# BornToDeath/h264-h265-to-jpeg

Hardware: AMD Instinct MI355X
Metric: 1080p H.265 I-frames/sec → JPEG at 1/2/4/8 MI355X; achieved HBM GB/s vs peak (higher is better)
Workload: dtype u8

## Files before the change

h264-h265-to-jpeg_amd/csrc/host/cabac.h:

```cpp
#pragma once
#include <cstdint>

namespace h2j {

#ifdef H2J_CABAC_COUNT
extern thread_local unsigned long long g_bins_ctx, g_bins_byp;
#define H2J_COUNT(v, n) (v += (n))
#else
#define H2J_COUNT(v, n) ((void)0)
#endif

#pragma GCC visibility push(hidden)
extern const uint8_t kCabacLps[64][4];
extern const uint8_t kCabacTransLps[64];
extern const uint8_t kCabacRenorm[32];
extern const uint16_t kCabacNextMps[128];
extern const uint16_t kCabacNextLps[128];
extern const uint8_t kCabacLpsByState[128][8];
typedef uint64_t CabacState;
extern const uint64_t kCabacWord[128];

extern const uint64_t kCabacNextMpsW[128];
extern const uint64_t kCabacNextLpsW[128];
#pragma GCC visibility pop


inline uint8_t cabac_init_state(int m, int n, int qp) {
    if (qp < 0) qp = 0;
    if (qp > 51) qp = 51;
    int pre = ((m * qp) >> 4) + n;
    if (pre < 1) pre = 1;
    if (pre > 126) pre = 126;
    int mps = pre <= 63 ? 0 : 1;
    int st = mps ? pre - 64 : 63 - pre;
    return static_cast<uint8_t>((st << 1) | mps);
}
inline CabacState cabac_init_word(int m, int n, int qp) { return kCabacWord[cabac_init_state(m, n, qp)]; }

template <bool kInlineRefill>
class CabacT {
public:
    void init(const uint8_t* p, const uint8_t* end) {
        cur_ = p;
        end_ = end;
        range_ = 510;
        value_ = 0;
        for (int i = 0; i < 4; i++) value_ = (value_ << 8) | (cur_ < end_ ? *cur_++ : 0u);
        bits_ = 32 - 9;
    }
    __attribute__((always_inline)) inline int decision(CabacState& ctx) {
        H2J_COUNT(g_bins_ctx, 1);
        const uint64_t w = ctx;
        const unsigned st = static_cast<unsigned>(w >> 32);
        const uint32_t lps = static_cast<uint32_t>(w >> ((range_ >> 3) & 24)) & 0xffu;
        const uint32_t rmps = range_ - lps;
        const uint64_t scaled = static_cast<uint64_t>(rmps) << bits_;
        const uint32_t msh = (rmps >> 8) ^ 1u;
        uint32_t r = rmps << msh, sh = msh;
        const uint32_t lsh = static_cast<uint32_t>(__builtin_clz(lps)) - 23u;
        const uint32_t lr = lps << lsh;
        uint64_t nx = kCabacNextMpsW[st];
        const uint64_t nl = kCabacNextLpsW[st];
        uint64_t v = value_;
        const uint64_t vl = value_ - scaled;
        uint32_t is_lps = 0;
#if defined(__x86_64__)
        __asm__("cmpq %[sc], %[v]\n\t"
                "cmovaeq %[vl], %[v]\n\t"
                "cmovael %[lr], %[r]\n\t"
                "cmovael %[ls], %[sh]\n\t"
                "cmovaeq %[nl], %[nx]\n\t"
                "setae %b[il]"
                : [v] "+r"(v), [r] "+r"(r), [sh] "+r"(sh), [nx] "+r"(nx), [il] "+q"(is_lps)
                : [sc] "r"(scaled), [vl] "r"(vl), [lr] "r"(lr), [ls] "r"(lsh), [nl] "r"(nl)
                : "cc");
#else
        is_lps = v >= scaled ? 1u : 0u;
        v = is_lps ? vl : v;
        r = is_lps ? lr : r;
        sh = is_lps ? lsh : sh;
        nx = is_lps ? nl : nx;
#endif
        value_ = v;
        range_ = r;
        bits_ -= static_cast<int>(sh);
        ctx = nx;
        if (bits_ < 0) refill();
        return static_cast<int>((st & 1) ^ is_lps);
    }
    __attribute__((always_inline)) int bypass_b() {
        H2J_COUNT(g_bins_byp, 1);
        if (--bits_ < 0) refill();
// ... 106 lines not shown
```

h264-h265-to-jpeg_amd/csrc/host/hevc_parser.cpp:

```cpp
#include <algorithm>
#include <array>
#include <atomic>
#include <cstdlib>
#include <cstring>
#include <memory>
#include <thread>
#include <vector>

#include "bitstream.h"
#include "cabac.h"
#include "job.h"

namespace h2j {
#ifdef H2J_CORO
extern thread_local void (*g_h2j_yield)();
#endif
namespace {

enum {
    C_SAO_MERGE = 0, C_SAO_TYPE = 1, C_SPLIT_CU = 2, C_TQ_BYPASS = 5, C_PART_MODE = 6,
    C_PREV_INTRA = 7, C_CHROMA_MODE = 8, C_SPLIT_TF = 9, C_CBF_LUMA = 12, C_CBF_CHROMA = 14,
    C_TSKIP = 18, C_LAST_X = 20, C_LAST_Y = 38, C_CSBF = 56, C_SIG = 60, C_GT1 = 104,
    C_GT2 = 128, C_QP_DELTA = 134, C_CQO_FLAG = 136, C_CQO_IDX = 137, NUM_CTX = 138
};

const uint8_t kInitI[NUM_CTX] = {
    153, 200, 139, 141, 157, 154, 184, 184, 63, 153, 138, 138, 111, 141, 94, 138, 182, 154,
    139, 139,
    110, 110, 124, 125, 140, 153, 125, 127, 140, 109, 111, 143, 127, 111, 79, 108, 123, 63,
    110, 110, 124, 125, 140, 153, 125, 127, 140, 109, 111, 143, 127, 111, 79, 108, 123, 63,
    91, 171, 134, 141,
    111, 111, 125, 110, 110, 94, 124, 108, 124, 107, 125, 141, 179, 153, 125, 107, 125, 141,
    179, 153, 125, 107, 125, 141, 179, 153, 125, 140, 139, 182, 182, 152, 136, 152, 136, 153,
    136, 139, 111, 136, 139, 111, 141, 111,
    140, 92, 137, 138, 140, 152, 138, 139, 153, 74, 149, 92, 139, 107, 122, 152, 140, 179, 166,
    182, 140, 227, 122, 197,
    138, 153, 136, 167, 152, 152,
    154, 154,
    154, 154};

struct Sps {
    bool valid = false;
    int chroma_format_idc = 0, width = 0, height = 0;
    int conf_l = 0, conf_r = 0, conf_t = 0, conf_b = 0;
    int bit_depth = 8, bit_depth_c = 8, log2_max_poc_lsb = 4;
    int num_reorder_pics = 0;
    int log2_min_cb = 3, log2_ctb = 4, log2_min_tb = 2, log2_max_tb = 5, max_th_depth_intra = 0;
    int scaling_list_enabled = 0;
    uint8_t sl[4][6][64];
    uint8_t sl_dc[4][6];
    int sao = 0, pcm = 0, pcm_bd = 8, pcm_bd_c = 8, log2_min_pcm = 0, log2_max_pcm = 0, pcm_lf_disabled = 0;
    int num_st_rps = 0;
    int st_num_delta[65];
    int long_term_present = 0, num_lt_sps = 0, temporal_mvp = 0, strong_intra_smoothing = 0;
    int profile_idc = 0;
    int ts_rotation = 0, ts_context = 0, implicit_rdpcm = 0, explicit_rdpcm = 0, ext_precision = 0;
    int smoothing_disabled = 0, high_prec_offsets = 0, persistent_rice = 0, bypass_alignment = 0;
};

struct Pps {
    bool valid = false;
    int sps_id = 0, dependent_slices = 0, output_flag_present = 0, num_extra_bits = 0, sign_hiding = 0;
    int init_qp = 26, transform_skip = 0, cu_qp_delta = 0, diff_cu_qp_delta_depth = 0;
    int cb_qp_offset = 0, cr_qp_offset = 0, slice_chroma_qp_present = 0, transquant_bypass = 0;
    int tiles = 0, wpp = 0, ntc = 1, ntr = 1, uniform = 1, lf_across_tiles = 1;
    int col_w[64], row_h[64];
    int lf_across_slices = 0, deblock_override = 0, deblock_disabled = 0, beta_offset = 0, tc_offset = 0;
    int sl_present = 0;
    uint8_t sl[4][6][64];
    uint8_t sl_dc[4][6];
    int slice_header_ext = 0;
    int log2_max_ts = 2, cross_component = 0, cqo_list_enabled = 0, sao_scale_luma = 0, sao_scale_chroma = 0;
    int cqo_depth = 0, cqo_len_minus1 = 0, cb_qo[6] = {0, 0, 0, 0, 0, 0}, cr_qo[6] = {0, 0, 0, 0, 0, 0};
};

struct SliceHdr {
    int first_in_pic = 0, dependent = 0, address = 0, slice_addr_rs = 0, pps_id = 0, type = 0;
    int sao_luma = 0, sao_chroma = 0, qp_delta = 0, cb_qp_offset = 0, cr_qp_offset = 0;
    int deblock_disabled = 0, beta_offset = 0, tc_offset = 0, lf_across_slices = 0, slice_qp = 26;
    int cu_chroma_qp_offset_enabled = 0;
    std::vector<uint32_t> entry;
};

const uint8_t kSlIntra[64] = {
    16, 16, 16, 16, 16, 16, 16, 16, 16, 16, 17, 16, 17, 16, 17, 18, 17, 18, 18, 17, 18, 21,
    19, 20, 21, 20, 19, 21, 24, 22, 22, 24, 24, 22, 22, 24, 25, 25, 27, 30, 27, 25, 25, 29,
    31, 35, 35, 31, 29, 36, 41, 44, 41, 36, 47, 54, 54, 47, 65, 70, 65, 88, 88, 115};
const uint8_t kSlInter[64] = {
    16, 16, 16, 16, 16, 16, 16, 16, 16, 16, 17, 17, 17, 17, 17, 18, 18, 18, 18, 18, 18, 20,
    20, 20, 20, 20, 20, 20, 24, 24, 24, 24, 24, 24, 24, 24, 25, 25, 25, 25, 25, 25, 25, 28,
    28, 28, 28, 28, 28, 33, 33, 33, 33, 33, 41, 41, 41, 41, 54, 54, 54, 71, 71, 91};

void sl_default(uint8_t sl[4][6][64], uint8_t dc[4][6]) {
    for (int m = 0; m < 6; m++) {
        std::memset(sl[0][m], 16, 16);
        for (int s = 1; s < 4; s++) {
            std::memcpy(sl[s][m], m < 3 ? kSlIntra : kSlInter, 64);
            dc[s][m] = 16;
        }
// ... 445 lines not shown
        ctbs_ = proto.ctbs_;
    }
    int run(const uint8_t* data, size_t size, int threads);

private:
    HevcParser(const HevcParser&) = default;
    FrameJob* job_;
    std::vector<h2j_ctb>* ctbs_;
    Sps sps_[16];
    Pps pps_[64];
    const Sps* s_ = nullptr;
    const Pps* p_ = nullptr;
    std::vector<SliceHdr> sh_;
    std::vector<uint8_t> rbsp_;
    std::vector<uint8_t> slice_data_;
    int W = 0, H = 0, log2ctb = 0, ctbs = 0, ctbW = 0, ctbH = 0, nctb = 0, mw = 0, mh = 0;
    int qpbd = 0;
    std::vector<int8_t> qp_store_;
    std::vector<uint8_t> ipm_store_, ctd_store_;
    std::vector<int> addr_store_, slice_store_;
    int8_t* qp_ = nullptr;
    uint8_t *ipm_ = nullptr, *ctd_ = nullptr;
    int *ctb_addr_rs_ = nullptr, *ctb_slice_ = nullptr;
    void bind_maps() {
        qp_ = qp_store_.data();
        ipm_ = ipm_store_.data();
        ctd_ = ctd_store_.data();
        ctb_addr_rs_ = addr_store_.data();
        ctb_slice_ = slice_store_.data();
    }
    std::vector<int> rs2ts_, ts2rs_, tile_id_, col_bd_;
    const SliceHdr* cur_ = nullptr;
    int cur_idx_ = 0;
    Cabac cc_;
    const uint8_t* end_ = nullptr;
    CabacState ctx_[NUM_CTX], ctx_wpp_[NUM_CTX], ctx_ds_[NUM_CTX];
    int stat_[4] = {0, 0, 0, 0}, stat_wpp_[4] = {0, 0, 0, 0}, stat_ds_[4] = {0, 0, 0, 0};
    bool rext_ = false;
    bool have_ds_ = false;
    int qp_y_ = 0, qg_pred_ = 0, qpd_val_ = 0, last_cu_qp_ = 0;
    bool is_qpd_coded_ = false, first_qg_ = true;
    bool cqo_coded_ = false;
    int cu_qo_cb_ = 0, cu_qo_cr_ = 0;
    int cu_bypass_ = 0;
    int cu_tu_begin_ = 0;
    int err_ = 0;

    int parse_slice_header(BitReader& b, int nal_type, SliceHdr& sh, const SliceHdr* prev);
    bool setup_picture();
    bool setup_tiles();
    int decode_slice_data(int shi, const uint8_t* p, const uint8_t* end);
    struct WppRows;
    int decode_wpp_row(int shi, int row, const uint8_t* p, const uint8_t* end, WppRows& w);
    int run_wpp(const std::vector<uint8_t>& seg, const std::vector<uint32_t>& sub, int threads);
    int decode_tile(int shi, int ts0, int ts1, bool last, const uint8_t* p, const uint8_t* end);
    int run_tiles(const std::vector<uint8_t>& seg, const std::vector<uint32_t>& sub, int threads);
    void merge_parts(const std::vector<FrameJob>& part);
    void ctb_start_contexts(int rs, int ts, bool first);
    void init_contexts(int qp) {
        for (int i = 0; i < NUM_CTX; i++) {
            int iv = kInitI[i];
            ctx_[i] = cabac_init_word((iv >> 4) * 5 - 45, ((iv & 15) << 3) - 16, qp);
        }
        std::memset(stat_, 0, sizeof(stat_));
    }
    bool same_region(int xc, int yc, int xn, int yn) const {
        if (xn < 0 || yn < 0 || xn >= W || yn >= H) return false;
        if (((xn ^ xc) | (yn ^ yc)) >> log2ctb == 0) return true;
        int cn = (yn >> log2ctb) * ctbW + (xn >> log2ctb);
        int cc = (yc >> log2ctb) * ctbW + (xc >> log2ctb);
        if (tile_id_[rs2ts_[cn]] != tile_id_[rs2ts_[cc]] || ctb_slice_[cn] < 0) return false;
        return ctb_addr_rs_[cn] == ctb_addr_rs_[cc];
    }
    void qg_start(int xq, int yq);
    void parse_sao(int rx, int ry);
    void coding_quadtree(int x0, int y0, int log2cb, int depth);
    void coding_unit(int x0, int y0, int log2cb);
    void transform_tree(int x0, int y0, int xb, int yb, int log2n, int depth, int blk, int max_depth,
                        int intra_split, int pcb, int pcr, int cm, int cux, int cuy, int log2cb);
    void transform_unit(int x0, int y0, int xb, int yb, int log2n, int blk, int cbf_l, int cbf_cb,
                        int cbf_cr, int cm, int cux, int cuy, int log2cb);
    template <bool RExt>
    void residual(int log2n, int c, int mode, h2j_tu& tu);
    void emit_tu(int x, int y, int log2n, int c, int mode, uint8_t flags, bool cbf, int pred_mode_for_scan);
    void split_ctb_records(size_t first);
    std::vector<h2j_tu> chroma_tmp_;
    uint8_t edge_flags(int x0, int y0) const;
    void pcm_sample(int x0, int y0, int log2cb);
    int qp_wrap(int x) const {
        const int m = 52 + qpbd;
        if (static_cast<unsigned>(x) < static_cast<unsigned>(2 * m)) return x >= m ? x - m : x;
        return x % m;
    }
    static void fill_rows(uint8_t* p, int stride, int rows, int w, uint8_t v) {
        const uint64_t v8 = 0x0101010101010101ull * v;
        for (int y = 0; y < rows; y++, p += stride) {
            if (w == 2) std::memcpy(p, &v8, 2);
            else if (w == 4) std::memcpy(p, &v8, 4);
            else if (w == 8) std::memcpy(p, &v8, 8);
            else if (w == 16) { std::memcpy(p, &v8, 8); std::memcpy(p + 8, &v8, 8); }
            else std::memset(p, v, static_cast<size_t>(w));
        }
    }
    void set_map(uint8_t* m, int x0, int y0, int n, uint8_t v) {
        int ye = std::min((y0 + n) >> 2, mh), xe = std::min((x0 + n) >> 2, mw);
        fill_rows(&m[(y0 >> 2) * mw + (x0 >> 2)], mw, ye - (y0 >> 2), xe - (x0 >> 2), v);
    }
    void set_qp(int x0, int y0, int n, int qp) {
        int ye = std::min((y0 + n) >> 2, mh), xe = std::min((x0 + n) >> 2, mw);
        fill_rows(reinterpret_cast<uint8_t*>(&qp_[(y0 >> 2) * mw + (x0 >> 2)]), mw, ye - (y0 >> 2), xe - (x0 >> 2),
                  static_cast<uint8_t>(qp & 0xFF));
    }
    __attribute__((always_inline)) int dec(int ctx) { return cc_.decision(ctx_[ctx]); }
};

int HevcParser::parse_slice_header(BitReader& b, int nal_type, SliceHdr& sh, const SliceHdr* prev) {
    sh = SliceHdr();
    sh.first_in_pic = static_cast<int>(b.u(1));
    if (nal_type >= 16 && nal_type <= 23) b.u(1);
    const uint32_t pps_id = b.ue();
    if (pps_id > 63 || !pps_[pps_id].valid) return -1;
    sh.pps_id = static_cast<int>(pps_id);
    const Pps& p = pps_[sh.pps_id];
    if (p.sps_id > 15 || !sps_[p.sps_id].valid) return -1;
    const Sps& s = sps_[p.sps_id];
    if (!sh.first_in_pic) {
        if (p.dependent_slices) sh.dependent = static_cast<int>(b.u(1));
        int cs = 1 << s.log2_ctb;
        int n = ((s.width + cs - 1) / cs) * ((s.height + cs - 1) / cs);
        sh.address = static_cast<int>(b.u(ceil_log2(n)));
        if (sh.address >= n) return -1;
    }
    if (sh.dependent) {
        if (!prev) return -1;
        int addr = sh.address, first = sh.first_in_pic;
        sh = *prev;
        sh.address = addr;
        sh.dependent = 1;
        sh.first_in_pic = first;
    } else {
        sh.slice_addr_rs = sh.address;
        for (int i = 0; i < p.num_extra_bits; i++) b.u(1);
        sh.type = static_cast<int>(b.ue());
        if (p.output_flag_present) b.u(1);
        if (nal_type != 19 && nal_type != 20) {
            b.u(s.log2_max_poc_lsb);
            int sps_flag = static_cast<int>(b.u(1));
            if (!sps_flag) {
                Sps tmp = s;
                if (!parse_st_rps(b, tmp, s.num_st_rps)) return -1;
            } else if (s.num_st_rps > 1) {
                b.u(ceil_log2(s.num_st_rps));
            }
            if (s.long_term_present) {
                uint32_t nsps = 0;
                if (s.num_lt_sps > 0) nsps = b.ue();
                const uint32_t npics = b.ue();
                if (nsps > static_cast<uint32_t>(s.num_lt_sps) || npics > 32) return -1;
                for (uint32_t i = 0; i < nsps + npics; i++) {
                    if (i < nsps) {
                        if (s.num_lt_sps > 1) b.u(ceil_log2(s.num_lt_sps));
                    } else {
                        b.u(s.log2_max_poc_lsb);
                        b.u(1);
                    }
                    if (b.u(1)) b.ue();
// ... 214 lines not shown
        std::memcpy(r.type, o.type, 3);
        std::memcpy(r.band_pos, o.band_pos, 3);
        std::memcpy(r.eo_class, o.eo_class, 3);
        std::memcpy(r.off, o.off, sizeof(r.off));
    };
    if (rx > 0) {
        int l = ctb - 1;
        if (tile_id_[rs2ts_[l]] == tile_id_[rs2ts_[ctb]] && ctb_slice_[l] >= 0 && ctb_addr_rs_[l] == ctb_addr_rs_[ctb]) {
            if (dec(C_SAO_MERGE)) { copy_from(l); return; }
        }
    }
    if (ry > 0) {
        int u = ctb - ctbW;
        if (tile_id_[rs2ts_[u]] == tile_id_[rs2ts_[ctb]] && ctb_slice_[u] >= 0 && ctb_addr_rs_[u] == ctb_addr_rs_[ctb]) {
            if (dec(C_SAO_MERGE)) { copy_from(u); return; }
        }
    }
    const int bd = s_->bit_depth;
    const int cmax = (1 << ((bd < 10 ? bd : 10) - 5)) - 1;
    for (int c = 0; c < 3; c++) {
        if ((c == 0 && !cur_->sao_luma) || (c > 0 && !cur_->sao_chroma)) continue;
        const int shift = c ? p_->sao_scale_chroma : p_->sao_scale_luma;
        if (c == 2) {
            r.type[2] = r.type[1];
            r.eo_class[2] = r.eo_class[1];
        } else {
            int t = 0;
            if (dec(C_SAO_TYPE)) t = cc_.bypass() ? 2 : 1;
            r.type[c] = static_cast<int8_t>(t);
        }
        if (r.type[c] == 0) continue;
        int a[4];
        for (int i = 0; i < 4; i++) {
            int v = 0;
            while (v < cmax && cc_.bypass()) v++;
            a[i] = v;
        }
        if (r.type[c] == 1) {
            for (int i = 0; i < 4; i++)
                if (a[i] && cc_.bypass()) a[i] = -a[i];
            r.band_pos[c] = static_cast<int8_t>(cc_.bypass_bits(5));
            for (int i = 0; i < 4; i++) r.off[c][i] = static_cast<int16_t>(a[i] * (1 << shift));
        } else {
            r.off[c][0] = static_cast<int16_t>(a[0] << shift);
            r.off[c][1] = static_cast<int16_t>(a[1] << shift);
            r.off[c][2] = static_cast<int16_t>(-(a[2] << shift));
            r.off[c][3] = static_cast<int16_t>(-(a[3] << shift));
            if (c == 0) r.eo_class[0] = static_cast<int8_t>(cc_.bypass_bits(2));
            if (c == 1) r.eo_class[1] = static_cast<int8_t>(cc_.bypass_bits(2));
        }
    }
}

uint8_t HevcParser::edge_flags(int x0, int y0) const {
    if (cur_->deblock_disabled) return 0;
    uint8_t f = 0;
    const int mask = ctbs - 1;
    if ((x0 & 7) == 0 && x0 > 0) {
        bool ok = true;
        if ((x0 & mask) == 0) {
            int cn = (y0 >> log2ctb) * ctbW + ((x0 - 1) >> log2ctb), cc = cn + 1;
            if (!cur_->lf_across_slices && ctb_addr_rs_[cn] != ctb_addr_rs_[cc]) ok = false;
            if (!p_->lf_across_tiles && tile_id_[rs2ts_[cn]] != tile_id_[rs2ts_[cc]]) ok = false;
        }
        if (ok) f |= H2J_TU_EDGE_L;
    }
    if ((y0 & 7) == 0 && y0 > 0) {
        bool ok = true;
        if ((y0 & mask) == 0) {
            int cc = (y0 >> log2ctb) * ctbW + (x0 >> log2ctb), cn = cc - ctbW;
            if (!cur_->lf_across_slices && ctb_addr_rs_[cn] != ctb_addr_rs_[cc]) ok = false;
            if (!p_->lf_across_tiles && tile_id_[rs2ts_[cn]] != tile_id_[rs2ts_[cc]]) ok = false;
        }
        if (ok) f |= H2J_TU_EDGE_T;
    }
    return f;
}

const uint8_t kSigTs[2][16] = {{C_SIG + 42, C_SIG + 42, C_SIG + 42, C_SIG + 42, C_SIG + 42, C_SIG + 42, C_SIG + 42, C_SIG + 42,
                                C_SIG + 42, C_SIG + 42, C_SIG + 42, C_SIG + 42, C_SIG + 42, C_SIG + 42, C_SIG + 42, C_SIG + 42},
                               {C_SIG + 43, C_SIG + 43, C_SIG + 43, C_SIG + 43, C_SIG + 43, C_SIG + 43, C_SIG + 43, C_SIG + 43,
                                C_SIG + 43, C_SIG + 43, C_SIG + 43, C_SIG + 43, C_SIG + 43, C_SIG + 43, C_SIG + 43, C_SIG + 43}};

template <bool RExt>
void HevcParser::residual(int log2n, int c, int pred_mode, h2j_tu& tu) {
    Cabac cc = cc_;
    CabacState* const ctx = ctx_;
    const int n = 1 << log2n;
    if (p_->transform_skip && !cu_bypass_ && log2n <= (RExt ? p_->log2_max_ts : 2) && cc.decision(ctx[C_TSKIP + (c ? 1 : 0)]))
        tu.flags |= H2J_TU_TSKIP;
    const bool tsb = (tu.flags & H2J_TU_TSKIP) != 0 || cu_bypass_;
    const bool ts_ctx = RExt && s_->ts_context && tsb;
    const bool no_sdh = RExt && s_->implicit_rdpcm && (tu.flags & H2J_TU_TSKIP) && (pred_mode == 10 || pred_mode == 26);
    const bool price = RExt && s_->persistent_rice;
    int* const stat = &stat_[2 * (c == 0 ? 1 : 0) + (tsb ? 1 : 0)];
    int off, shift;
    if (c == 0) {
        off = 3 * (log2n - 2) + ((log2n - 1) >> 2);
        shift = (log2n + 1) >> 2;
    } else {
        off = 15;
        shift = log2n - 2;
    }
    const int maxp = (log2n << 1) - 1;
    auto last_prefix = [&](CabacState* lc) __attribute__((always_inline)) {
        int k = 0, pk = 0;
        CabacState pw = lc[0];
        while (k < maxp) {
            const int ci = k >> shift;
            const CabacState lw = lc[ci];
            lc[pk] = pw;
            CabacState w = ci == pk ? pw : lw;
            const int b = cc.decision(w);
            pw = w;
            pk = ci;
            if (!b) break;
            k++;
        }
        lc[pk] = pw;
        return k;
    };
    int lx = last_prefix(ctx + C_LAST_X + off);
    int ly = last_prefix(ctx + C_LAST_Y + off);
    if (lx > 3) {
        int nb = (lx >> 1) - 1;
        lx = (1 << nb) * (2 + (lx & 1)) + static_cast<int>(cc.bypass_bits(nb));
    }
    if (ly > 3) {
        int nb = (ly >> 1) - 1;
        ly = (1 << nb) * (2 + (ly & 1)) + static_cast<int>(cc.bypass_bits(nb));
    }
    int scanIdx = 0;
    if (log2n == 2 || (log2n == 3 && c == 0)) {
        if (pred_mode >= 6 && pred_mode <= 14) scanIdx = 2;
        else if (pred_mode >= 22 && pred_mode <= 30) scanIdx = 1;
    }
    if (scanIdx == 2) std::swap(lx, ly);
    if (lx >= n || ly >= n) { err_ = -20; cc_ = cc; return; }
    const uint8_t(*sc)[64][2] = scanIdx == 0 ? g_scan_diag : (scanIdx == 1 ? g_scan_hor : g_scan_ver);
    const int lsb = log2n - 2;
    const int lastSub = g_scan_inv[scanIdx][lsb][((ly >> 2) << lsb) + (lx >> 2)];
    const int lastPos = g_scan_inv[scanIdx][2][((ly & 3) << 2) + (lx & 3)];
    uint8_t csbf[8][8];
    std::memset(csbf, 0, sizeof(csbf));
    int greater1_ctx = 1;
    const bool sdh = p_->sign_hiding != 0;
    const int sbw = 1 << lsb;
    uint32_t out[32 * 32];
    int nout = 0;
    const uint16_t* const posTab = g_scan_off[scanIdx][lsb];
    const uint8_t(*const sigtab)[2][16] = g_sigctx[c ? 1 : 0][lsb][scanIdx];
    CabacState* const gt1ctx = ctx + C_GT1 + (c ? 16 : 0);
    for (int i = lastSub; i >= 0; i--) {
#ifdef H2J_CORO_SB
        if (i < lastSub && g_h2j_yield) g_h2j_yield();
#endif
        const int xs = sc[lsb][i][0], ys = sc[lsb][i][1];
        bool infer_dc = false;
        if (i < lastSub && i > 0) {
            int csr = (xs + 1 < sbw) ? csbf[xs + 1][ys] : 0;
            int csb = (ys + 1 < sbw) ? csbf[xs][ys + 1] : 0;
            csbf[xs][ys] = static_cast<uint8_t>(cc.decision(ctx[C_CSBF + (csr | csb) + (c ? 2 : 0)]));
            infer_dc = true;
        } else {
            csbf[xs][ys] = 1;
        }
        unsigned sigmask = 0;
        int nstart = 15;
        if (i == lastSub) {
            nstart = lastPos - 1;
            sigmask = 1u << lastPos;
        }
        if (csbf[xs][ys]) {
            int prevCsbf = 0;
            if (xs + 1 < sbw) prevCsbf |= csbf[xs + 1][ys];
            if (ys + 1 < sbw) prevCsbf |= csbf[xs][ys + 1] << 1;
            const uint8_t* sig = ts_ctx ? kSigTs[c ? 1 : 0] : sigtab[prevCsbf][(xs | ys) ? 1 : 0];
            unsigned got = 0;
            if (nstart > 0) {
                int pidx = sig[nstart];
                CabacState pw = ctx[pidx];
                got = static_cast<unsigned>(cc.decision(pw)) << nstart;
                for (int nn = nstart - 1; nn > 0; nn--) {
                    const int idx = sig[nn];
                    const CabacState lw = ctx[idx];
                    ctx[pidx] = pw;
                    CabacState w = idx == pidx ? pw : lw;
                    got |= static_cast<unsigned>(cc.decision(w)) << nn;
                    pw = w;
                    pidx = idx;
                }
                ctx[pidx] = pw;
            }
            sigmask |= got;
            infer_dc = infer_dc && got == 0;
            if (nstart >= 0) {
                if (!infer_dc) {
                    if (cc.decision(ctx[sig[0]])) sigmask |= 1u;
                } else {
                    sigmask |= 1u;
                }
            }
        }
        if (!sigmask) continue;
        int ctxSet = (i == 0 || c > 0) ? 0 : 2;
        if (greater1_ctx == 0) ctxSet++;
        greater1_ctx = 1;
        unsigned g1mask = 0;
        int numG1 = 0, lastG1 = -1;
        unsigned m_uncoded = 0;
        const int lastSig = 31 - __builtin_clz(sigmask), firstSig = __builtin_ctz(sigmask);
        CabacState* const g1c = gt1ctx + ctxSet * 4;
        {
            CabacState w0 = g1c[0], w1 = g1c[1], w2 = g1c[2], w3 = g1c[3];
            unsigned seen = 0, m = sigmask;
            auto bin = [&](CabacState& slot) __attribute__((always_inline)) {
                const int nn = 31 - __builtin_clz(m);
                m &= ~(1u << nn);
                CabacState w = seen ? w0 : slot;
                const unsigned d = static_cast<unsigned>(cc.decision(w));
                if (seen) w0 = w;
                else slot = w;
                seen |= d;
                g1mask |= d << nn;
                numG1++;
            };
            if (m) bin(w1);
            if (m) bin(w2);
            while (m && numG1 < 8) bin(w3);
            g1c[0] = w0;
            g1c[1] = w1;
            g1c[2] = w2;
            g1c[3] = w3;
            m_uncoded = m;
            greater1_ctx = seen ? 0 : 1;
        }
        if (g1mask) lastG1 = 31 - __builtin_clz(g1mask);
        const bool hidden = !cu_bypass_ && !no_sdh && (lastSig - firstSig > 3);
        int g2 = 0;
        if (lastG1 != -1) g2 = cc.decision(ctx[C_GT2 + ctxSet + (c ? 4 : 0)]);
        const unsigned signed_mask = (sdh && hidden) ? (sigmask & ~(1u << firstSig)) : sigmask;
        const int ns = __builtin_popcount(signed_mask);
        const uint32_t q = ns > 1 ? cc.bypass_batch(ns) : (ns ? static_cast<uint32_t>(cc.bypass()) : 0u);
        uint32_t qs = ns ? q << (32 - ns) : 0u;
        unsigned esc = g1mask | m_uncoded;
        if (lastG1 >= 0 && !g2) esc &= ~(1u << lastG1);
        int remv[16] = {};
        int rice = price ? *stat / 4 : 0;
        bool stat_done = false;
        for (unsigned e = esc; e;) {
            const int nn = 31 - __builtin_clz(e);
            e &= ~(1u << nn);
            const int baseL = 1 + ((g1mask >> nn) & 1) + (nn == lastG1 ? g2 : 0);
            {
                constexpr int kPeek = 20;
                const uint32_t q = cc.bypass_peek(kPeek);
                const uint32_t inv = ~q << (32 - kPeek);
                int prefix = inv ? __builtin_clz(inv) : kPeek;
                int rem = -1;
                if (prefix < kPeek) {
                    const int slen = prefix < 3 ? rice : prefix - 3 + rice, total = prefix + 1 + slen;
                    if (total <= kPeek) {
                        const uint32_t top = q >> (kPeek - total);
                        cc.bypass_skip(total, top);
                        const int suf = static_cast<int>(top & ((1u << slen) - 1u));
                        rem = prefix < 3 ? (prefix << rice) + suf : (((1 << (prefix - 3)) + 2) << rice) + suf;
                    }
                }
                if (rem < 0) {
                    prefix = 0;
                    while (prefix < 32 && cc.bypass()) prefix++;
                    if (prefix < 3) rem = (prefix << rice) + static_cast<int>(cc.bypass_bits(rice));
                    else {
                        int pm3 = prefix - 3;
                        if (pm3 + rice > 30) { err_ = -21; cc_ = cc; return; }
                        rem = (((1 << pm3) + 2) << rice) + static_cast<int>(cc.bypass_bits(pm3 + rice));
                    }
                }
                remv[nn] = rem;
                if (baseL + rem > 3 * (1 << rice)) rice = price ? rice + 1 : (rice < 4 ? rice + 1 : 4);
                if (price && !stat_done) {
                    const int ri = *stat / 4;
                    if (rem >= (3 << ri)) ++*stat;
                    else if (2 * rem < (1 << ri) && *stat > 0) --*stat;
                    stat_done = true;
                }
            }
        }
        const int flip_last = (sdh && hidden) ? 1 : 0;
        const int sb_off = ((ys << 2) << log2n) + (xs << 2);
        int sumAbs = 0;
        for (unsigned mm = sigmask; mm;) {
            const int nn = 31 - __builtin_clz(mm);
            mm &= ~(1u << nn);
            const int lvl = 1 + ((g1mask >> nn) & 1) + (nn == lastG1 ? g2 : 0) + remv[nn];
            sumAbs += lvl;
            const int neg = static_cast<int>(qs >> 31) ^ (mm == 0 ? (flip_last & sumAbs) : 0);
            qs <<= 1;
            int v = neg ? -lvl : lvl;
            if (v > 32767) v = 32767;
            if (v < -32768) v = -32768;
            out[nout++] = (static_cast<uint32_t>(sb_off + posTab[nn]) << 16) | static_cast<uint16_t>(v);
        }
    }
    cc_ = cc;
    const uint32_t base = static_cast<uint32_t>(job_->coefs.size());
    job_->coefs.insert(job_->coefs.end(), out, out + nout);
    tu.coef = base - job_->hdr.coef;
    tu.ncoef = static_cast<uint16_t>(nout);
    tu.flags |= H2J_TU_CBF;
}

void HevcParser::split_ctb_records(size_t first) {
    std::vector<h2j_tu>& v = job_->tus;
    chroma_tmp_.clear();
    size_t w = first;
    for (size_t i = first; i < v.size(); i++) {
        if (v[i].c == 0) v[w++] = v[i];
        else chroma_tmp_.push_back(v[i]);
    }
    std::copy(chroma_tmp_.begin(), chroma_tmp_.end(), v.begin() + static_cast<long>(w));
}

void HevcParser::emit_tu(int x, int y, int log2n, int c, int mode, uint8_t flags, bool cbf, int) {
    job_->tus.emplace_back();
    h2j_tu& tu = job_->tus.back();
    tu.x = static_cast<uint16_t>(x);
    tu.y = static_cast<uint16_t>(y);
    tu.log2n = static_cast<uint8_t>(log2n);
    tu.c = static_cast<uint8_t>(c);
    tu.mode = static_cast<uint8_t>(mode);
    tu.flags = flags;
    tu.qp = 0;
    tu.qpy = 0;
    tu.ncoef = 0;
    tu.coef = 0;
    if (cbf) {
#ifdef H2J_CORO
        if (g_h2j_yield) g_h2j_yield();
#endif
        if (rext_) residual<true>(log2n, c, mode, tu);
        else residual<false>(log2n, c, mode, tu);
    }
}

void HevcParser::transform_unit(int x0, int y0, int xb, int yb, int log2n, int blk, int cbf_l, int cbf_cb,
                                int cbf_cr, int cm, int cux, int cuy, int log2cb) {
    if ((cbf_l || cbf_cb || cbf_cr) && p_->cu_qp_delta && !is_qpd_coded_) {
        int v = 0;
        if (dec(C_QP_DELTA)) {
            v = 1;
            while (v < 5 && dec(C_QP_DELTA + 1)) v++;
            if (v == 5) {
                int k = 0;
                while (k < 32 && cc_.bypass()) k++;
                if (k > 30) { err_ = -22; return; }
                v += ((1 << k) - 1) + static_cast<int>(cc_.bypass_bits(k));
            }
        }
        if (v && cc_.bypass()) v = -v;
        is_qpd_coded_ = true;
        qpd_val_ = v;
        qp_y_ = qp_wrap(qg_pred_ + v + 52 + 2 * qpbd) - qpbd;
        set_qp(cux, cuy, 1 << log2cb, qp_y_);
    }
    if ((cbf_cb || cbf_cr) && cur_->cu_chroma_qp_offset_enabled && !cu_bypass_ && !cqo_coded_) {
        int idx = -1;
        if (dec(C_CQO_FLAG)) {
            idx = 0;
            if (p_->cqo_len_minus1 > 0)
                while (idx < 5 && dec(C_CQO_IDX)) idx++;
        }
        cu_qo_cb_ = idx < 0 ? 0 : p_->cb_qo[idx];
        cu_qo_cr_ = idx < 0 ? 0 : p_->cr_qo[idx];
        cqo_coded_ = true;
    }
    const int lmode = ipm_[(y0 >> 2) * mw + (x0 >> 2)];
    uint8_t fl = edge_flags(x0, y0);
    if (cu_bypass_) fl |= H2J_TU_BYPASS | H2J_TU_NOFILT;
    uint8_t lfl = fl;
    if (log2n == 2) lfl |= H2J_TU_DST;
    emit_tu(x0, y0, log2n, 0, lmode, lfl, cbf_l != 0, lmode);
    if ((job_->tus.back().flags & (H2J_TU_TSKIP | H2J_TU_BYPASS)) != 0) job_->tus.back().flags &= ~H2J_TU_DST;
    if (err_) return;
    uint8_t cfl = cu_bypass_ ? (H2J_TU_BYPASS | H2J_TU_NOFILT) : 0;
    if (log2n > 2) {
        emit_tu(x0 >> 1, y0 >> 1, log2n - 1, 1, cm, cfl, cbf_cb != 0, cm);
        if (err_) return;
        emit_tu(x0 >> 1, y0 >> 1, log2n - 1, 2, cm, cfl, cbf_cr != 0, cm);
    } else if (blk == 3) {
        emit_tu(xb >> 1, yb >> 1, 2, 1, cm, cfl, cbf_cb != 0, cm);
        if (err_) return;
        emit_tu(xb >> 1, yb >> 1, 2, 2, cm, cfl, cbf_cr != 0, cm);
    }
}

void HevcParser::transform_tree(int x0, int y0, int xb, int yb, int log2n, int depth, int blk, int max_depth,
                                int intra_split, int pcb, int pcr, int cm, int cux, int cuy, int log2cb) {
    if (err_) return;
    int split;
    if (log2n <= s_->log2_max_tb && log2n > s_->log2_min_tb && depth < max_depth && !(intra_split && depth == 0))
        split = dec(C_SPLIT_TF + 5 - log2n);
    else
        split = log2n > s_->log2_max_tb || (intra_split && depth == 0);
    int cbf_cb = 0, cbf_cr = 0;
    if (log2n > 2) {
        if (depth == 0 || pcb) cbf_cb = dec(C_CBF_CHROMA + depth);
        if (depth == 0 || pcr) cbf_cr = dec(C_CBF_CHROMA + depth);
    } else {
        cbf_cb = pcb;
        cbf_cr = pcr;
    }
    if (split) {
        if (log2n <= 2) { err_ = -23; return; }
        int h = 1 << (log2n - 1);
        transform_tree(x0, y0, x0, y0, log2n - 1, depth + 1, 0, max_depth, intra_split, cbf_cb, cbf_cr, cm, cux, cuy, log2cb);
        transform_tree(x0 + h, y0, x0, y0, log2n - 1, depth + 1, 1, max_depth, intra_split, cbf_cb, cbf_cr, cm, cux, cuy, log2cb);
        transform_tree(x0, y0 + h, x0, y0, log2n - 1, depth + 1, 2, max_depth, intra_split, cbf_cb, cbf_cr, cm, cux, cuy, log2cb);
        transform_tree(x0 + h, y0 + h, x0, y0, log2n - 1, depth + 1, 3, max_depth, intra_split, cbf_cb, cbf_cr, cm, cux, cuy, log2cb);
    } else {
        int cbf_l = dec(C_CBF_LUMA + (depth == 0 ? 1 : 0));
        transform_unit(x0, y0, xb, yb, log2n, blk, cbf_l, cbf_cb, cbf_cr, cm, cux, cuy, log2cb);
    }
// ... 575 lines not shown
```

Before: 2076.

## Add single-coefficient subblock fast path and bitmask CSBF in HEVC residual parsing

Replaces the 8x8 coded-sub-block flag array with a 64-bit mask and derives neighbour flags with shifts, avoiding a memset and branchy lookups. Adds a fast path for sub-blocks with exactly one significant coefficient that decodes gt1/gt2/sign and an out-of-line remaining level directly, skipping the generic multi-coefficient machinery. Factors remaining-level decoding into a shared inline helper, uses bypass_bits for small sign counts, and removes coroutine yield hooks. It also adds compile-time residual statistics counters that are off by default. The fast path must reproduce the generic path's context, sign-hiding and rice update behaviour exactly, which carries a correctness risk.

```diff
diff --git a/h264-h265-to-jpeg_amd/csrc/host/cabac.h b/h264-h265-to-jpeg_amd/csrc/host/cabac.h
--- a/h264-h265-to-jpeg_amd/csrc/host/cabac.h
+++ b/h264-h265-to-jpeg_amd/csrc/host/cabac.h
@@ -6,8 +6,17 @@
 #ifdef H2J_CABAC_COUNT
 extern thread_local unsigned long long g_bins_ctx, g_bins_byp;
 #define H2J_COUNT(v, n) (v += (n))
+struct ResidualStats {
+    unsigned long long tbs, sb_visited, csbf_bins, sb_coded, sig_bins, sig0_bins, gt1_bins, gt2_bins, last_bins,
+        coefs, sb_by_coefs[5] , rem_coefs, rem_sbs, sign_batch_sbs, sign_single_sbs;
+    unsigned long long one_coef, one_coef_esc, one_coef_esc_price, one_coef_tskip, one_coef_bypass, one_coef_esc_tskip,
+        one_coef_esc_bypass, dc_last_sb, dc_only_tb, sign_pair;
+};
+extern thread_local ResidualStats g_rstat;
+#define H2J_STAT(f, n) (g_rstat.f += (n))
 #else
 #define H2J_COUNT(v, n) ((void)0)
+#define H2J_STAT(f, n) ((void)0)
 #endif
 
 #pragma GCC visibility push(hidden)
diff --git a/h264-h265-to-jpeg_amd/csrc/host/hevc_parser.cpp b/h264-h265-to-jpeg_amd/csrc/host/hevc_parser.cpp
--- a/h264-h265-to-jpeg_amd/csrc/host/hevc_parser.cpp
+++ b/h264-h265-to-jpeg_amd/csrc/host/hevc_parser.cpp
@@ -12,9 +12,6 @@
 #include "job.h"
 
 namespace h2j {
-#ifdef H2J_CORO
-extern thread_local void (*g_h2j_yield)();
-#endif
 namespace {
 
 enum {
@@ -626,6 +623,7 @@
                         int cbf_cr, int cm, int cux, int cuy, int log2cb);
     template <bool RExt>
     void residual(int log2n, int c, int mode, h2j_tu& tu);
+    int remaining_level(int rice);
     void emit_tu(int x, int y, int log2n, int c, int mode, uint8_t flags, bool cbf, int pred_mode_for_scan);
     void split_ctb_records(size_t first);
     std::vector<h2j_tu> chroma_tmp_;
@@ -1006,6 +1004,30 @@
                                {C_SIG + 43, C_SIG + 43, C_SIG + 43, C_SIG + 43, C_SIG + 43, C_SIG + 43, C_SIG + 43, C_SIG + 43,
                                 C_SIG + 43, C_SIG + 43, C_SIG + 43, C_SIG + 43, C_SIG + 43, C_SIG + 43, C_SIG + 43, C_SIG + 43}};
 
+__attribute__((always_inline)) inline int read_remaining(Cabac& cc, int rice) {
+    constexpr int kPeek = 20;
+    const uint32_t q = cc.bypass_peek(kPeek);
+    const uint32_t inv = ~q << (32 - kPeek);
+    int prefix = inv ? __builtin_clz(inv) : kPeek;
+    if (prefix < kPeek) {
+        const int slen = prefix < 3 ? rice : prefix - 3 + rice, total = prefix + 1 + slen;
+        if (total <= kPeek) {
+            const uint32_t top = q >> (kPeek - total);
+            cc.bypass_skip(total, top);
+            const int suf = static_cast<int>(top & ((1u << slen) - 1u));
+            return prefix < 3 ? (prefix << rice) + suf : (((1 << (prefix - 3)) + 2) << rice) + suf;
+        }
+    }
+    prefix = 0;
+    while (prefix < 32 && cc.bypass()) prefix++;
+    if (prefix < 3) return (prefix << rice) + static_cast<int>(cc.bypass_bits(rice));
+    const int pm3 = prefix - 3;
+    if (pm3 + rice > 30) return -1;
+    return (((1 << pm3) + 2) << rice) + static_cast<int>(cc.bypass_bits(pm3 + rice));
+}
+
+__attribute__((noinline)) int HevcParser::remaining_level(int rice) { return read_remaining(cc_, rice); }
+
 template <bool RExt>
 void HevcParser::residual(int log2n, int c, int pred_mode, h2j_tu& tu) {
     Cabac cc = cc_;
@@ -1027,6 +1049,7 @@
         shift = log2n - 2;
     }
     const int maxp = (log2n << 1) - 1;
+    H2J_STAT(tbs, 1);
     auto last_prefix = [&](CabacState* lc) __attribute__((always_inline)) {
         int k = 0, pk = 0;
         CabacState pw = lc[0];
@@ -1035,6 +1058,7 @@
             const CabacState lw = lc[ci];
             lc[pk] = pw;
             CabacState w = ci == pk ? pw : lw;
+            H2J_STAT(last_bins, 1);
             const int b = cc.decision(w);
             pw = w;
             pk = ci;
@@ -1065,43 +1089,42 @@
     const int lsb = log2n - 2;
     const int lastSub = g_scan_inv[scanIdx][lsb][((ly >> 2) << lsb) + (lx >> 2)];
     const int lastPos = g_scan_inv[scanIdx][2][((ly & 3) << 2) + (lx & 3)];
-    uint8_t csbf[8][8];
-    std::memset(csbf, 0, sizeof(csbf));
+    uint64_t csbm = 0;
+    H2J_STAT(dc_only_tb, (lx | ly) == 0);
     int greater1_ctx = 1;
     const bool sdh = p_->sign_hiding != 0;
-    const int sbw = 1 << lsb;
     uint32_t out[32 * 32];
     int nout = 0;
     const uint16_t* const posTab = g_scan_off[scanIdx][lsb];
     const uint8_t(*const sigtab)[2][16] = g_sigctx[c ? 1 : 0][lsb][scanIdx];
     CabacState* const gt1ctx = ctx + C_GT1 + (c ? 16 : 0);
     for (int i = lastSub; i >= 0; i--) {
-#ifdef H2J_CORO_SB
-        if (i < lastSub && g_h2j_yield) g_h2j_yield();
-#endif
         const int xs = sc[lsb][i][0], ys = sc[lsb][i][1];
+        H2J_STAT(sb_visited, 1);
         bool infer_dc = false;
+        const int sp = ys * 8 + xs;
+        const unsigned csr = static_cast<unsigned>(((csbm >> 1) & 0x7f7f7f7f7f7f7f7full) >> sp) & 1u;
+        const unsigned csb = static_cast<unsigned>((csbm >> 8) >> sp) & 1u;
+        unsigned coded = 1;
         if (i < lastSub && i > 0) {
-            int csr = (xs + 1 < sbw) ? csbf[xs + 1][ys] : 0;
-            int csb = (ys + 1 < sbw) ? csbf[xs][ys + 1] : 0;
-            csbf[xs][ys] = static_cast<uint8_t>(cc.decision(ctx[C_CSBF + (csr | csb) + (c ? 2 : 0)]));
+            H2J_STAT(csbf_bins, 1);
+            coded = static_cast<unsigned>(cc.decision(ctx[C_CSBF + (csr | csb) + (c ? 2 : 0)]));
             infer_dc = true;
-        } else {
-            csbf[xs][ys] = 1;
-        }
+        }
+        csbm |= static_cast<uint64_t>(coded) << sp;
+        const int prevCsbf = static_cast<int>(csr | (csb << 1));
         unsigned sigmask = 0;
         int nstart = 15;
         if (i == lastSub) {
             nstart = lastPos - 1;
             sigmask = 1u << lastPos;
-        }
-        if (csbf[xs][ys]) {
-            int prevCsbf = 0;
-            if (xs + 1 < sbw) prevCsbf |= csbf[xs + 1][ys];
-            if (ys + 1 < sbw) prevCsbf |= csbf[xs][ys + 1] << 1;
+            H2J_STAT(dc_last_sb, lastPos == 0);
+        }
+        if (coded && nstart >= 0) {
             const uint8_t* sig = ts_ctx ? kSigTs[c ? 1 : 0] : sigtab[prevCsbf][(xs | ys) ? 1 : 0];
             unsigned got = 0;
             if (nstart > 0) {
+                H2J_STAT(sig_bins, nstart);
                 int pidx = sig[nstart];
                 CabacState pw = ctx[pidx];
                 got = static_cast<unsigned>(cc.decision(pw)) << nstart;
@@ -1117,18 +1140,64 @@
                 ctx[pidx] = pw;
             }
             sigmask |= got;
-            infer_dc = infer_dc && got == 0;
-            if (nstart >= 0) {
-                if (!infer_dc) {
-                    if (cc.decision(ctx[sig[0]])) sigmask |= 1u;
-                } else {
-                    sigmask |= 1u;
-                }
+            if (infer_dc && got == 0) {
+                sigmask |= 1u;
+            } else {
+                H2J_STAT(sig0_bins, 1);
+                if (cc.decision(ctx[sig[0]])) sigmask |= 1u;
             }
         }
         if (!sigmask) continue;
+        H2J_STAT(sb_coded, 1);
         int ctxSet = (i == 0 || c > 0) ? 0 : 2;
         if (greater1_ctx == 0) ctxSet++;
+        const int sb_off = ((ys << 2) << log2n) + (xs << 2);
+#ifdef H2J_CABAC_COUNT
+        {
+            const int nc = __builtin_popcount(sigmask);
+            H2J_STAT(coefs, nc);
+            H2J_STAT(sb_by_coefs[nc == 1 ? 0 : nc == 2 ? 1 : nc == 3 ? 2 : nc < 8 ? 3 : 4], 1);
+            H2J_STAT(gt1_bins, nc < 8 ? nc : 8);
+        }
+#endif
+        if ((sigmask & (sigmask - 1)) == 0) {
+            H2J_STAT(one_coef, 1);
+            H2J_STAT(sign_single_sbs, 1);
+            H2J_STAT(one_coef_tskip, (tu.flags & H2J_TU_TSKIP) != 0);
+            H2J_STAT(one_coef_bypass, cu_bypass_ != 0);
+            const int g1 = cc.decision(gt1ctx[ctxSet * 4 + 1]);
+            greater1_ctx = g1 ^ 1;
+            int lvl = 1 + g1, g2 = 0;
+            if (g1) {
+                H2J_STAT(gt2_bins, 1);
+                g2 = cc.decision(ctx[C_GT2 + ctxSet + (c ? 4 : 0)]);
+                lvl += g2;
+            }
+            const int neg = cc.bypass();
+            if (g2) {
+                H2J_STAT(one_coef_esc, 1);
+                H2J_STAT(one_coef_esc_price, price);
+                H2J_STAT(one_coef_esc_tskip, (tu.flags & H2J_TU_TSKIP) != 0);
+                H2J_STAT(one_coef_esc_bypass, cu_bypass_ != 0);
+                H2J_STAT(rem_coefs, 1);
+                H2J_STAT(rem_sbs, 1);
+                cc_ = cc;
+                const int rem = remaining_level(price ? *stat / 4 : 0);
+                cc = cc_;
+                if (rem < 0) { err_ = -21; return; }
+                lvl += rem;
+                if (price) {
+                    const int ri = *stat / 4;
+                    if (rem >= (3 << ri)) ++*stat;
+                    else if (2 * rem < (1 << ri) && *stat > 0) --*stat;
+                }
+            }
+            int v = neg ? -lvl : lvl;
+            if (v > 32767) v = 32767;
+            if (v < -32768) v = -32768;
+            out[nout++] = (static_cast<uint32_t>(sb_off + posTab[__builtin_ctz(sigmask)]) << 16) | static_cast<uint16_t>(v);
+            continue;
+        }
         greater1_ctx = 1;
         unsigned g1mask = 0;
         int numG1 = 0, lastG1 = -1;
@@ -1162,13 +1231,21 @@
         if (g1mask) lastG1 = 31 - __builtin_clz(g1mask);
         const bool hidden = !cu_bypass_ && !no_sdh && (lastSig - firstSig > 3);
         int g2 = 0;
-        if (lastG1 != -1) g2 = cc.decision(ctx[C_GT2 + ctxSet + (c ? 4 : 0)]);
+        if (lastG1 != -1) {
+            H2J_STAT(gt2_bins, 1);
+            g2 = cc.decision(ctx[C_GT2 + ctxSet + (c ? 4 : 0)]);
+        }
         const unsigned signed_mask = (sdh && hidden) ? (sigmask & ~(1u << firstSig)) : sigmask;
         const int ns = __builtin_popcount(signed_mask);
-        const uint32_t q = ns > 1 ? cc.bypass_batch(ns) : (ns ? static_cast<uint32_t>(cc.bypass()) : 0u);
+        H2J_STAT(sign_batch_sbs, ns > 1);
+        H2J_STAT(sign_single_sbs, ns <= 1);
+        H2J_STAT(sign_pair, ns == 2);
+        const uint32_t q = ns > 2 ? cc.bypass_batch(ns) : cc.bypass_bits(ns);
         uint32_t qs = ns ? q << (32 - ns) : 0u;
         unsigned esc = g1mask | m_uncoded;
         if (lastG1 >= 0 && !g2) esc &= ~(1u << lastG1);
+        H2J_STAT(rem_coefs, __builtin_popcount(esc));
+        H2J_STAT(rem_sbs, esc != 0);
         int remv[16] = {};
         int rice = price ? *stat / 4 : 0;
         bool stat_done = false;
@@ -1176,43 +1253,18 @@
             const int nn = 31 - __builtin_clz(e);
             e &= ~(1u << nn);
             const int baseL = 1 + ((g1mask >> nn) & 1) + (nn == lastG1 ? g2 : 0);
-            {
-                constexpr int kPeek = 20;
-                const uint32_t q = cc.bypass_peek(kPeek);
-                const uint32_t inv = ~q << (32 - kPeek);
-                int prefix = inv ? __builtin_clz(inv) : kPeek;
-                int rem = -1;
-                if (prefix < kPeek) {
-                    const int slen = prefix < 3 ? rice : prefix - 3 + rice, total = prefix + 1 + slen;
-                    if (total <= kPeek) {
-                        const uint32_t top = q >> (kPeek - total);
-                        cc.bypass_skip(total, top);
-                        const int suf = static_cast<int>(top & ((1u << slen) - 1u));
-                        rem = prefix < 3 ? (prefix << rice) + suf : (((1 << (prefix - 3)) + 2) << rice) + suf;
-                    }
-                }
-                if (rem < 0) {
-                    prefix = 0;
-                    while (prefix < 32 && cc.bypass()) prefix++;
-                    if (prefix < 3) rem = (prefix << rice) + static_cast<int>(cc.bypass_bits(rice));
-                    else {
-                        int pm3 = prefix - 3;
-                        if (pm3 + rice > 30) { err_ = -21; cc_ = cc; return; }
-                        rem = (((1 << pm3) + 2) << rice) + static_cast<int>(cc.bypass_bits(pm3 + rice));
-                    }
-                }
-                remv[nn] = rem;
-                if (baseL + rem > 3 * (1 << rice)) rice = price ? rice + 1 : (rice < 4 ? rice + 1 : 4);
-                if (price && !stat_done) {
-                    const int ri = *stat / 4;
-                    if (rem >= (3 << ri)) ++*stat;
-                    else if (2 * rem < (1 << ri) && *stat > 0) --*stat;
-                    stat_done = true;
-                }
+            const int rem = read_remaining(cc, rice);
+            if (rem < 0) { err_ = -21; cc_ = cc; return; }
+            remv[nn] = rem;
+            if (baseL + rem > 3 * (1 << rice)) rice = price ? rice + 1 : (rice < 4 ? rice + 1 : 4);
+            if (price && !stat_done) {
+                const int ri = *stat / 4;
+                if (rem >= (3 << ri)) ++*stat;
+                else if (2 * rem < (1 << ri) && *stat > 0) --*stat;
+                stat_done = true;
             }
         }
         const int flip_last = (sdh && hidden) ? 1 : 0;
-        const int sb_off = ((ys << 2) << log2n) + (xs << 2);
         int sumAbs = 0;
         for (unsigned mm = sigmask; mm;) {
             const int nn = 31 - __builtin_clz(mm);
@@ -1260,9 +1312,6 @@
     tu.ncoef = 0;
     tu.coef = 0;
     if (cbf) {
-#ifdef H2J_CORO
-        if (g_h2j_yield) g_h2j_yield();
-#endif
         if (rext_) residual<true>(log2n, c, mode, tu);
         else residual<false>(log2n, c, mode, tu);
     }
```

Measured after the change: 2166 (median of 6 runs). 1.04x the previous value.
